# Baverne/VAE-CYCLEGAN-Implementation

Hardware: AMD Instinct MI355X
Metric: train images/sec (256x256 VAE-CycleGAN step) (higher is better)
Workload: dtype f32; 1 GPU; cyclevaegan unpaired, 3x256x256 synthetic summer<->winter, per-GPU batch 8, latent 64 (BASELINE.json configs[3]/[4]); per_gpu_batch=8, global_batch=8, image_size=256, latent_dim=64, parallelism=dp1, init=random (reference init statistics)

## Files before the change

vae-cyclegan-implementation_amd/csrc/conv_wino.hip:

```cpp
#include "vcg_common.h"
#ifdef VCG_STAMP
#include <stdlib.h>
#endif

#define WINO_U_SHIFT 2
#define WINO_V_SHIFT 2
int vcg_gemm_planes_batched(const void* APlanes, const void* BtPlanes, float* C, int rows, int K, int N, int batches, const VcgAmax& amax_a,
                            const VcgAmax& amax_b, hipStream_t st, uint32_t* amax_a_keep);

struct WinoP {
  const float* x;
  const float* m;
  const float* bias;
  float* y;
  int N, H, W, Cin, Cout, Hl, Wl, ups, reflect, act, cout_log;
  int th, tw, T, Kc;
  int off;
  FastDiv fd_k4, fd_tw, fd_thtw, fd_c4, fd_co4;
  unsigned long long* amax_slot;
  uint32_t amax_gen;
  VcgAmax amax_x;
  unsigned short* vplanes;
  const float* pre_mean;
  const float* pre_rstd;
  int pre_act;
};
__device__ __forceinline__ float4 wino_pre_apply(const float4& v, const float4& mu, const float4& rs, int act) {
  return make_float4(act_apply((v.x - mu.x) * rs.x, act), act_apply((v.y - mu.y) * rs.y, act), act_apply((v.z - mu.z) * rs.z, act),
                     act_apply((v.w - mu.w) * rs.w, act));
}

__device__ __forceinline__ float4 f4sub(const float4& a, const float4& b) { return make_float4(a.x - b.x, a.y - b.y, a.z - b.z, a.w - b.w); }
__device__ __forceinline__ float4 f4sum(const float4& a, const float4& b) { return make_float4(a.x + b.x, a.y + b.y, a.z + b.z, a.w + b.w); }

__global__ __launch_bounds__(256) void k_wino_in_planes(WinoP p) {
  float sc, inv;
  vcg_scale_of(vcg_amax_bits(p.amax_x), p.amax_x.shift, sc, inv);
  const uint32_t k4n = (uint32_t)p.Kc / 4;
  const size_t total = (size_t)p.T * k4n;
  const size_t KB = (size_t)p.Kc / 32;
  for (size_t idx = (size_t)blockIdx.x * blockDim.x + threadIdx.x; idx < total; idx += (size_t)gridDim.x * blockDim.x) {
// ... 377 lines not shown
  const size_t plane = (size_t)p.T * p.Cout;
  for (size_t idx = (size_t)blockIdx.x * blockDim.x + threadIdx.x; idx < total; idx += (size_t)gridDim.x * blockDim.x) {
    const uint32_t t = (uint32_t)(idx / c4n);
    const int co = (int)(idx - (size_t)t * c4n) * 4;
    const uint32_t n = fd_div(t, p.fd_thtw);
    const uint32_t rem = t - n * (uint32_t)(p.th * p.tw);
    const uint32_t ty = fd_div(rem, p.fd_tw);
    const int tx = (int)(rem - ty * (uint32_t)p.tw);
    const float* base = dy + (((size_t)n * p.Hl + 2 * ty) * p.Wl + 2 * tx) * p.Cout + co;
    const float4 y00 = *reinterpret_cast<const float4*>(base);
    const float4 y01 = *reinterpret_cast<const float4*>(base + p.Cout);
    const float4 y10 = *reinterpret_cast<const float4*>(base + (size_t)p.Wl * p.Cout);
    const float4 y11 = *reinterpret_cast<const float4*>(base + (size_t)p.Wl * p.Cout + p.Cout);
    const float4 zero = make_float4(0.f, 0.f, 0.f, 0.f);
    float4 z[4][2];
    z[0][0] = y00;              z[0][1] = y01;
    z[1][0] = f4sum(y00, y10);  z[1][1] = f4sum(y01, y11);
    z[2][0] = f4sub(y00, y10);  z[2][1] = f4sub(y01, y11);
    z[3][0] = f4sub(zero, y10); z[3][1] = f4sub(zero, y11);
    float* mb = dm + (size_t)t * p.Cout + co;
#pragma unroll
    for (int a = 0; a < 4; ++a) {
      const float4 o1 = f4sum(z[a][0], z[a][1]), o2 = f4sub(z[a][0], z[a][1]);
      *reinterpret_cast<float4*>(mb + (size_t)(a * 4 + 0) * plane) = z[a][0];
      *reinterpret_cast<float4*>(mb + (size_t)(a * 4 + 1) * plane) = o1;
      *reinterpret_cast<float4*>(mb + (size_t)(a * 4 + 2) * plane) = o2;
      *reinterpret_cast<float4*>(mb + (size_t)(a * 4 + 3) * plane) = f4sub(zero, z[a][1]);
      amax = max(amax, max(max(vcg_abs_bits4(z[a][0]), vcg_abs_bits4(z[a][1])), max(vcg_abs_bits4(o1), vcg_abs_bits4(o2))));
    }
  }
  if (p.amax_slot) vcg_amax_publish(amax, p.amax_slot, p.amax_gen, amax_red);
}

constexpr int WT_PITCH = 34;
__device__ __forceinline__ void wino_tr_store(unsigned short* __restrict__ sh, const float4* __restrict__ o4, float inv, int tl, int q,
                                              unsigned short* __restrict__ dst, size_t xi_stride, size_t row0, int TB, int tb) {
#pragma unroll
  for (int x = 0; x < 4; ++x) {
    uint2 h, l;
    split4h(o4[x], inv, h, l);
    const unsigned short hv[4] = {(unsigned short)h.x, (unsigned short)(h.x >> 16), (unsigned short)h.y, (unsigned short)(h.y >> 16)};
    const unsigned short lv[4] = {(unsigned short)l.x, (unsigned short)(l.x >> 16), (unsigned short)l.y, (unsigned short)(l.y >> 16)};
#pragma unroll
    for (int e = 0; e < 4; ++e) {
      sh[((x * 2 + 0) * 32 + 4 * q + e) * WT_PITCH + tl] = hv[e];
      sh[((x * 2 + 1) * 32 + 4 * q + e) * WT_PITCH + tl] = lv[e];
    }
  }
  __syncthreads();
  {
    const int pc = threadIdx.x & 1, c = (threadIdx.x >> 1) & 31, x = threadIdx.x >> 6;
    const uint32_t* src = reinterpret_cast<const uint32_t*>(sh + ((x * 2 + pc) * 32 + c) * WT_PITCH);
    uint4 v[4];
#pragma unroll
    for (int j = 0; j < 4; ++j) v[j] = make_uint4(src[4 * j], src[4 * j + 1], src[4 * j + 2], src[4 * j + 3]);
    unsigned short* o = dst + (size_t)x * xi_stride + ((row0 + c) * TB + tb) * VCG_PBLK + pc * 32;
#pragma unroll
    for (int j = 0; j < 4; ++j) *reinterpret_cast<uint4*>(o + 8 * j) = v[j];
  }
  __syncthreads();
}
__global__ __launch_bounds__(256) void k_wino_in_tr(WinoP p, unsigned short* __restrict__ vt) {
  __shared__ __attribute__((aligned(16))) unsigned short sh[4 * 2 * 32 * WT_PITCH];
  float sc, inv;
  vcg_scale_of(vcg_amax_bits(p.amax_x), p.amax_x.shift, sc, inv);
  const int tl = threadIdx.x >> 3, q = threadIdx.x & 7;
  const uint32_t t = blockIdx.x * 32 + tl;
  const uint32_t k4 = blockIdx.y * 8 + q;
  const uint32_t ph = fd_div(k4, p.fd_c4);
  const int c = (int)(k4 - ph * (uint32_t)(p.Cin / 4)) * 4;
  const int pi = (int)(ph >> 1), pj = (int)(ph & 1);
  const uint32_t n = fd_div(t, p.fd_thtw);
  const uint32_t rem = t - n * (uint32_t)(p.th * p.tw);
  const uint32_t ty = fd_div(rem, p.fd_tw);
  const int tx = (int)(rem - ty * (uint32_t)p.tw);
  const float* xn = p.x + (size_t)n * p.H * p.W * p.Cin;
  float4 pmu = make_float4(0.f, 0.f, 0.f, 0.f), prs = pmu;
  if (p.pre_mean) {
    pmu = *reinterpret_cast<const float4*>(p.pre_mean + (size_t)n * p.Cin + c);
    prs = *reinterpret_cast<const float4*>(p.pre_rstd + (size_t)n * p.Cin + c);
  }
  float4 d[4][4];
#pragma unroll
  for (int r = 0; r < 4; ++r) {
    int ih = 2 * (int)ty - p.off + r;
    bool okh = true;
    if (p.reflect) ih = reflect_idx(ih, p.Hl);
    else okh = ih >= 0 && ih < p.Hl;
#pragma unroll
    for (int s = 0; s < 4; ++s) {
      int iw = 2 * tx - p.off + s;
      bool ok = okh;
      if (p.reflect) iw = reflect_idx(iw, p.Wl);
      else ok = ok && iw >= 0 && iw < p.Wl;
      d[r][s] = ok ? *reinterpret_cast<const float4*>(xn + ((size_t)(ih * p.ups + pi) * p.W + (iw * p.ups + pj)) * p.Cin + c)
                   : make_float4(0.f, 0.f, 0.f, 0.f);
      if (p.pre_mean && ok) d[r][s] = wino_pre_apply(d[r][s], pmu, prs, p.pre_act);
    }
  }
  float4 e[4][4];
#pragma unroll
  for (int s = 0; s < 4; ++s) {
    e[0][s] = f4sub(d[0][s], d[2][s]);
    e[1][s] = f4sum(d[1][s], d[2][s]);
    e[2][s] = f4sub(d[2][s], d[1][s]);
    e[3][s] = f4sub(d[1][s], d[3][s]);
  }
  const uint32_t k = k4 * 4;
  const size_t KB = (size_t)p.Kc / 32;
  const int TB = p.T / 32;
#pragma unroll
  for (int a = 0; a < 4; ++a) {
    const float4 o[4] = {f4sub(e[a][0], e[a][2]), f4sum(e[a][1], e[a][2]), f4sub(e[a][2], e[a][1]), f4sub(e[a][1], e[a][3])};
    if (p.vplanes) {
      unsigned short* vb = p.vplanes + ((size_t)t * KB + k / 32) * VCG_PBLK + (k & 31);
      const size_t plane = (size_t)p.T * KB * VCG_PBLK;
#pragma unroll
      for (int b = 0; b < 4; ++b) {
        uint2 h, l;
        split4h(o[b], inv, h, l);
        unsigned short* w = vb + (size_t)(a * 4 + b) * plane;
        *reinterpret_cast<uint2*>(w) = h;
        *reinterpret_cast<uint2*>(w + 32) = l;
      }
    }
    if (vt) wino_tr_store(sh, o, inv, tl, q, vt + (size_t)(a * 4) * p.Kc * TB * VCG_PBLK, (size_t)p.Kc * TB * VCG_PBLK, (size_t)blockIdx.y * 32, TB, (int)blockIdx.x);
  }
}
__global__ __launch_bounds__(256) void k_wino_dy_tr(const float* __restrict__ dy, unsigned short* __restrict__ dmt, WinoP p) {
  __shared__ __attribute__((aligned(16))) unsigned short sh[4 * 2 * 32 * WT_PITCH];
  float sc, inv;
  vcg_scale_of(vcg_amax_bits(p.amax_x), p.amax_x.shift, sc, inv);
  const int tl = threadIdx.x >> 3, q = threadIdx.x & 7;
  const uint32_t t = blockIdx.x * 32 + tl;
  const int co = ((int)blockIdx.y * 8 + q) * 4;
  const uint32_t n = fd_div(t, p.fd_thtw);
  const uint32_t rem = t - n * (uint32_t)(p.th * p.tw);
  const uint32_t ty = fd_div(rem, p.fd_tw);
  const int tx = (int)(rem - ty * (uint32_t)p.tw);
  const float* base = dy + (((size_t)n * p.Hl + 2 * ty) * p.Wl + 2 * tx) * p.Cout + co;
  const float4 y00 = *reinterpret_cast<const float4*>(base);
  const float4 y01 = *reinterpret_cast<const float4*>(base + p.Cout);
  const float4 y10 = *reinterpret_cast<const float4*>(base + (size_t)p.Wl * p.Cout);
  const float4 y11 = *reinterpret_cast<const float4*>(base + (size_t)p.Wl * p.Cout + p.Cout);
  const float4 zero = make_float4(0.f, 0.f, 0.f, 0.f);
  float4 z[4][2];
  z[0][0] = y00;              z[0][1] = y01;
  z[1][0] = f4sum(y00, y10);  z[1][1] = f4sum(y01, y11);
  z[2][0] = f4sub(y00, y10);  z[2][1] = f4sub(y01, y11);
  z[3][0] = f4sub(zero, y10); z[3][1] = f4sub(zero, y11);
  const int TB = p.T / 32;
#pragma unroll
  for (int a = 0; a < 4; ++a) {
    const float4 o[4] = {z[a][0], f4sum(z[a][0], z[a][1]), f4sub(z[a][0], z[a][1]), f4sub(zero, z[a][1])};
    wino_tr_store(sh, o, inv, tl, q, dmt + (size_t)(a * 4) * p.Cout * TB * VCG_PBLK, (size_t)p.Cout * TB * VCG_PBLK, (size_t)blockIdx.y * 32, TB, (int)blockIdx.x);
  }
}

static int wino_blocks(size_t work) {
  size_t b = (work + 255) / 256;
  if (b > 8192) b = 8192;
  return b < 1 ? 1 : (int)b;
}

bool vcg_wino_weight_ok(const ConvGeom& g) {
  return g.KH == 3 && g.KW == 3 && g.stride == 1 && g.pad == 1 && g.ups * g.ups * g.Cin >= 128 && g.Cout >= 64 &&
         g.Cin % 4 == 0 && g.Cout % 64 == 0 && (g.ups * g.ups * g.Cin) % 64 == 0;
}
static bool wino_map_ok(const ConvGeom& g) {
  if (!vcg_wino_weight_ok(g)) return false;
#ifdef VCG_STAMP
  if (getenv("VCG_NO_WINOGRAD")) return false;
#endif
  return !(g.Ho < 4 || g.Wo < 4 || (g.Ho & 1) || (g.Wo & 1));
}
bool vcg_wino_fwd_ok(const ConvGeom& g) {
  if (!wino_map_ok(g)) return false;
  const unsigned long long T = (unsigned long long)g.N * (g.Ho / 2) * (g.Wo / 2);
  const unsigned long long Kc = (unsigned long long)g.ups * g.ups * g.Cin;
  if (Kc * g.Cout < (unsigned long long)kWinoGateFwd * (Kc + g.Cout)) return false;
  return T * Kc * 4 < (1ull << 31) && T * g.Cout * 4 < (1ull << 31) && T * Kc * 16 < (1ull << 32);
}
size_t vcg_wino_weight_floats(const ConvGeom& g) { return (size_t)16 * g.ups * g.ups * g.Cin * g.Cout * VCG_NP / 2; }
size_t vcg_wino_fwd_workspace(const ConvGeom& g) {
  const size_t T = (size_t)g.N * (g.Ho / 2) * (g.Wo / 2);
  return (size_t)16 * T * ((size_t)g.ups * g.ups * g.Cin + g.Cout) * sizeof(float) + 512;
}
int vcg_wino_weight(const ConvGeom& g, const float* w_oihw, float* u, const VcgAmax& amax_w, hipStream_t st) {
// ... 16 lines not shown
  p.fd_co4 = make_fastdiv((uint32_t)g.Cout / 4);
  p.off = 1;
  p.amax_slot = nullptr; p.amax_gen = 0;
  p.amax_x = vcg_amax_const(0); p.vplanes = nullptr;
  p.pre_mean = nullptr; p.pre_rstd = nullptr; p.pre_act = VCG_ACT_NONE;
  return p;
}

bool vcg_wino_wgrad_ok(const ConvGeom& g) {
  const long long kc = (long long)g.ups * g.ups * g.Cin;
  return vcg_wino_fwd_ok(g) && kc % 128 == 0 && kc * g.Cout >= kWinoGateWgrad * (kc + g.Cout);
}
bool vcg_wino_wgrad_tr_ok(const ConvGeom& g) {
  if (!vcg_wino_wgrad_ok(g)) return false;
  const long long kc = (long long)g.ups * g.ups * g.Cin, T = (long long)g.N * (g.Ho / 2) * (g.Wo / 2);
  return T % 32 == 0 && kc % 32 == 0 && g.Cout % 128 == 0 && kc >= 256 && ((kc + 255) / 256) * (g.Cout / 128) * 16 >= 192 &&
         16 * kc * T * VCG_NP < (1ll << 32) && 16 * (long long)g.Cout * T * VCG_NP < (1ll << 32);
}
size_t vcg_wino_wgrad_workspace(const ConvGeom& g) {
  const int T = g.N * (g.Ho / 2) * (g.Wo / 2);
  return vcg_wino_fwd_workspace(g) + vcg_wino_wgrad_core_workspace(g, T);
}
static size_t wino_v_floats(const ConvGeom& g) { return (size_t)16 * g.N * (g.Ho / 2) * (g.Wo / 2) * g.ups * g.ups * g.Cin; }
size_t vcg_wino_saved_floats(const ConvGeom& g) { return vcg_wino_wgrad_ok(g) ? wino_v_floats(g) + 16 : 0; }
int vcg_wino_wgrad(const ConvGeom& g, const float* x, const float* dy, float* gw_oihw, void* ws, size_t ws_bytes, hipStream_t st,
                   const float* v_saved, uint64_t x_handle, uint64_t dy_handle) {
  VCG_CHECK_ARG(ws && ws_bytes >= vcg_wino_wgrad_workspace(g), "vcg_conv_wgrad: workspace too small for the Winograd path");
  WinoP p = wino_params(g);
  float* V = (float*)ws;
  float* dM = V + (((size_t)16 * p.T * p.Kc + 63) / 64) * 64;
  const size_t tbytes = vcg_wino_fwd_workspace(g);
  if (vcg_wino_wgrad_tr_ok(g)) {
    VcgAmax amax_v;
    const unsigned short* Vt;
    if (v_saved) {
      Vt = reinterpret_cast<const unsigned short*>(v_saved);
      amax_v = vcg_amax_stored(v_saved + wino_v_floats(g), WINO_V_SHIFT);
    } else {
      if (vcg_operand_amax(x, (size_t)g.N * g.H * g.W * g.Cin, x_handle, WINO_V_SHIFT, st, &amax_v)) return -2;
      p.x = x; p.amax_x = amax_v; p.vplanes = nullptr;
      hipLaunchKernelGGL(k_wino_in_tr, dim3(p.T / 32, p.Kc / 32), dim3(256), 0, st, p, (unsigned short*)V);
      Vt = reinterpret_cast<const unsigned short*>(V);
    }
    VcgAmax amax_d;
    if (vcg_operand_amax(dy, (size_t)g.N * g.Ho * g.Wo * g.Cout, dy_handle, WINO_V_SHIFT, st, &amax_d)) return -2;
    WinoP pd = p;
    pd.amax_x = amax_d;
    hipLaunchKernelGGL(k_wino_dy_tr, dim3(p.T / 32, g.Cout / 32), dim3(256), 0, st, dy, (unsigned short*)dM, pd);
    VCG_LAUNCH_CHECK("vcg_conv_wgrad(winograd transforms, transposed)");
    float* dU = reinterpret_cast<float*>((char*)ws + tbytes);
    if (vcg_gemm_planes_batched(Vt, dM, dU, p.Kc, p.T, g.Cout, 16, amax_v, amax_d, st, nullptr)) return -2;
    return vcg_wino_wgrad_reduce_one(g, dU, gw_oihw, st);
  }
  p.x = x;
  VcgAmax amax_v;
  if (v_saved) {
    V = const_cast<float*>(v_saved);
    amax_v = vcg_amax_stored(v_saved + wino_v_floats(g), WINO_V_SHIFT);
  } else {
    if (vcg_operand_amax(x, (size_t)g.N * g.H * g.W * g.Cin, x_handle, WINO_V_SHIFT, st, &amax_v)) return -2;
    p.amax_x = amax_v; p.vplanes = (unsigned short*)V;
    hipLaunchKernelGGL(k_wino_in_planes, dim3(wino_blocks((size_t)p.T * p.Kc / 4)), dim3(256), 0, st, p);
  }
  const VcgAmaxOut ad = vcg_amax_new(st);
  p.amax_slot = ad.slot; p.amax_gen = ad.gen;
  hipLaunchKernelGGL(k_wino_dy, dim3(wino_blocks((size_t)p.T * g.Cout / 4)), dim3(256), 0, st, dy, dM, p);
  VCG_LAUNCH_CHECK("vcg_conv_wgrad(winograd transforms)");
  return vcg_wino_wgrad_core(g, V, dM, p.T, gw_oihw, (char*)ws + tbytes, ws_bytes - tbytes, st, amax_v, vcg_amax_in(ad));
}

bool vcg_wino_dgrad_ok(const ConvGeom& g) {
  if (!wino_map_ok(g)) return false;
  const long long kc = (long long)g.ups * g.ups * g.Cin;
  if (kc * g.Cout < kWinoGateDgrad * (kc + g.Cout)) return false;
  const unsigned long long Tp = (unsigned long long)g.N * (g.Ho / 2 + 1) * (g.Wo / 2 + 1);
  return Tp * kc * 4 < (1ull << 31) && Tp * g.Cout * 4 < (1ull << 31) && Tp * g.Cout * 16 < (1ull << 32);
}
size_t vcg_wino_dgrad_workspace(const ConvGeom& g) {
  const size_t Tp = (size_t)g.N * (g.Ho / 2 + 1) * (g.Wo / 2 + 1);
  const size_t kc = (size_t)g.ups * g.ups * g.Cin;
  return (size_t)16 * Tp * (kc + g.Cout) * sizeof(float) + 1024;
}
int vcg_wino_weight_dgrad(const ConvGeom& g, const float* w_oihw, float* ud, const VcgAmax& amax_w, hipStream_t st) {
  const size_t total = (size_t)g.ups * g.ups * g.Cin * g.Cout / 4;
// ... 24 lines not shown
  if (vcg_operand_amax(dy, (size_t)g.N * g.Ho * g.Wo * g.Cout, dy_handle, WINO_V_SHIFT, st, &ad)) return -2;
  p.amax_x = ad; p.vplanes = (unsigned short*)V;
  hipLaunchKernelGGL(k_wino_in_planes, dim3(wino_blocks((size_t)p.T * g.Cout / 4)), dim3(256), 0, st, p);
  VCG_LAUNCH_CHECK("vcg_conv_dgrad(winograd input transform)");
  if (vcg_gemm_planes_batched(V, ud, M, p.T, g.Cout, kc, 16, ad, vcg_amax_stored(w_amax, WINO_U_SHIFT), st, nullptr)) return -2;
  WinoP q = p;
  q.Kc = kc;
  hipLaunchKernelGGL(k_wino_out_fold, dim3(wino_blocks((size_t)p.T * kc / 4)), dim3(256), 0, st, (const float*)M, dx, q, g.Hl, g.Wl,
                     g.Cin, g.ups, g.reflect);
  VCG_LAUNCH_CHECK("vcg_conv_dgrad(winograd output transform)");
  return 0;
}

size_t vcg_wino_fwd_stats_doubles(const ConvGeom& g) {
  const NormPlan pl = vcg_norm_plan(g.N, (g.Ho / 2) * (g.Wo / 2), g.Cout);
  return (size_t)g.N * pl.nchunk * g.Cout * 2;
}
int vcg_wino_fwd(const ConvGeom& g, const float* x, const float* u, const void* w_amax, const float* bias, float* y, void* ws,
                 size_t ws_bytes, hipStream_t st, double* in_part, const VcgInStatsOut* stats, float* v_keep, uint64_t x_handle,
                 const VcgPre* pre) {
  VCG_CHECK_ARG(ws && ws_bytes >= vcg_wino_fwd_workspace(g), "vcg_conv_fwd: workspace too small for the Winograd path (%zu)",
                ws_bytes);
  WinoP p = wino_params(g);
  float* V = v_keep ? v_keep : (float*)ws;
  float* M = (float*)ws + (((size_t)16 * p.T * p.Kc + 63) / 64) * 64;
  p.x = x; p.m = M; p.bias = bias; p.y = y;
  uint32_t pre_bits = 0;
  if (pre && pre->mean) {
    p.pre_mean = pre->mean; p.pre_rstd = pre->rstd; p.pre_act = pre->act;
    const float bound = sqrtf((float)g.H * (float)g.W);
    memcpy(&pre_bits, &bound, 4);
  }
  uint32_t* const keep_word = v_keep ? reinterpret_cast<uint32_t*>(v_keep + wino_v_floats(g)) : nullptr;
  if (v_keep && vcg_wino_wgrad_tr_ok(g)) {
    VcgAmax ax;
    if (pre_bits) ax = vcg_amax_const(pre_bits, WINO_V_SHIFT);
    else if (vcg_operand_amax(x, (size_t)g.N * g.H * g.W * g.Cin, x_handle, WINO_V_SHIFT, st, &ax)) return -2;
    V = (float*)ws;
    p.amax_x = ax; p.vplanes = (unsigned short*)V;
    hipLaunchKernelGGL(k_wino_in_tr, dim3(p.T / 32, p.Kc / 32), dim3(256), 0, st, p, (unsigned short*)v_keep);
    VCG_LAUNCH_CHECK("vcg_conv_fwd(winograd input transform, + transposed)");
    if (vcg_gemm_planes_batched(V, u, M, p.T, p.Kc, g.Cout, 16, ax, vcg_amax_stored(w_amax, WINO_U_SHIFT), st, keep_word)) return -2;
  } else {
    VcgAmax ax;
    if (pre_bits) ax = vcg_amax_const(pre_bits, WINO_V_SHIFT);
    else if (vcg_operand_amax(x, (size_t)g.N * g.H * g.W * g.Cin, x_handle, WINO_V_SHIFT, st, &ax)) return -2;
    p.amax_x = ax; p.vplanes = (unsigned short*)V;
    hipLaunchKernelGGL(k_wino_in_planes, dim3(wino_blocks((size_t)p.T * p.Kc / 4)), dim3(256), 0, st, p);
    VCG_LAUNCH_CHECK("vcg_conv_fwd(winograd input transform)");
    if (vcg_gemm_planes_batched(V, u, M, p.T, p.Kc, g.Cout, 16, ax, vcg_amax_stored(w_amax, WINO_U_SHIFT), st, keep_word)) return -2;
  }
  if (in_part) {
    const NormPlan pl = vcg_norm_plan(g.N, p.th * p.tw, g.Cout);
    hipLaunchKernelGGL(k_wino_out_stats, dim3(pl.nchunk, g.N, pl.cgroups), dim3(256), 0, st, p, in_part, pl);
    VCG_LAUNCH_CHECK("vcg_conv_fwd(winograd output transform)");
    return vcg_in_finalize(in_part, stats->mean, stats->rstd, g.N, stats->HW, g.Cout, pl.nchunk, stats->eps, st);
  } else {
    hipLaunchKernelGGL(k_wino_out, dim3(wino_blocks((size_t)p.T * g.Cout / 4)), dim3(256), 0, st, p);
  }
  VCG_LAUNCH_CHECK("vcg_conv_fwd(winograd output transform)");
  return 0;
}
```

vae-cyclegan-implementation_amd/csrc/gemm_split.hip:

```cpp
#include "vcg_common.h"

typedef unsigned int u32x4g __attribute__((ext_vector_type(4)));

struct GemmSplitP {
  const float* a;
  const float* bt;
  float* c;
  int rows, K, N;
  uint32_t a_bytes, b_bytes;
  uint32_t a_bstride, b_bstride;
  size_t c_bstride;
  VcgAmax amax_a, amax_b;
  uint32_t* amax_a_keep;
};

#define GS_OOB 0x80000000u

template <int BN>
__global__ __launch_bounds__(256, 2) void k_gemm_split(GemmSplitP p) {
  constexpr int BM = 128, NI = BN / 64, MI = 2;
  __shared__ __attribute__((aligned(16))) unsigned char As[VCG_NP][BM * 64];
  __shared__ __attribute__((aligned(16))) unsigned char Bs[VCG_NP][BN * 64];
  const int tid = threadIdx.x, lane = tid & 63, wid = tid >> 6;
  const int wm = wid >> 1, wn = wid & 1, l31 = lane & 31, lh = lane >> 5;
// ... 116 lines not shown

struct GdSrd { uint32_t x, y, z, w; };
typedef uint32_t gd_u32x4 __attribute__((ext_vector_type(4)));
__device__ __forceinline__ gd_u32x4 gd_srd(const void* ptr, uint32_t bytes) {
  const uint64_t a = (uint64_t)ptr;
  gd_u32x4 r;
  r.x = __builtin_amdgcn_readfirstlane((uint32_t)a);
  r.y = __builtin_amdgcn_readfirstlane((uint32_t)(a >> 32) & 0xFFFFu);
  r.z = __builtin_amdgcn_readfirstlane(bytes);
  r.w = 0x00020000u;
  return r;
}
__device__ __forceinline__ void gd_dma16(gd_u32x4 srd, uint32_t lds_dst, uint32_t voff) {
  uint32_t keep;
  asm volatile("s_mov_b32 %0, m0\n\ts_mov_b32 m0, %2\n\ts_nop 0\n\tbuffer_load_dwordx4 %1, %3, 0 offen lds\n\ts_mov_b32 m0, %0"
               : "=&s"(keep) : "v"(voff), "s"(lds_dst), "s"(srd) : "memory");
}
__device__ __forceinline__ void gd_barrier() {
  asm volatile("s_waitcnt lgkmcnt(0)\n\ts_barrier" ::: "memory");
}
constexpr int GD_BM = 256, GD_BN = 128;
constexpr int GD_A_BYTES = GD_BM * VCG_PBYTES, GD_B_BYTES = GD_BN * VCG_PBYTES;
constexpr int GD_STAGE = GD_A_BYTES + GD_B_BYTES;
constexpr int GD_STAGES = 3;
#ifdef VCG_GD_STAMP
__device__ unsigned long long* g_gd_stamp = nullptr;
int vcg_gd_set_stamp(void* buf) { return hipMemcpyToSymbol(HIP_SYMBOL(g_gd_stamp), &buf, sizeof(buf)) == hipSuccess ? 0 : -1; }
#define GD_T() (__builtin_amdgcn_sched_barrier(0), __builtin_amdgcn_s_memtime())
#define GD_ACC(slot, t0) do { const unsigned long long t1__ = GD_T(); gd_acc[slot] += t1__ - (t0); (t0) = t1__; } while (0)
#else
#define GD_T() 0ull
#define GD_ACC(slot, t0) do { } while (0)
#endif
__global__ __launch_bounds__(512, 1) void k_gemm_planes_dma(GemmSplitP p) {
  __shared__ __attribute__((aligned(1024))) unsigned char smem[GD_STAGES * GD_STAGE];
  const int tid = threadIdx.x, lane = tid & 63, wid = tid >> 6;
  const int wm = wid >> 1, wn = wid & 1;
  float sa_, inv_a, sb_, inv_b;
  {
    const uint32_t abits = vcg_amax_bits(p.amax_a);
    vcg_scale_of(abits, p.amax_a.shift, sa_, inv_a);
    vcg_scale_of(vcg_amax_bits(p.amax_b), p.amax_b.shift, sb_, inv_b);
    if (p.amax_a_keep && tid == 0 && blockIdx.x == 0 && blockIdx.y == 0 && blockIdx.z == 0) *p.amax_a_keep = abits;
  }
  int mt, nt, zb;
  {
    const uint32_t per = gridDim.x * gridDim.y, nwg = per * gridDim.z;
    const uint32_t gid = blockIdx.x + gridDim.x * (blockIdx.y + gridDim.y * blockIdx.z);
    const uint32_t q = nwg >> 3, r = nwg & 7, xcd = gid & 7;
    const uint32_t swz = (xcd < r ? xcd * (q + 1) : r * (q + 1) + (xcd - r) * q) + (gid >> 3);
    zb = (int)(swz / per);
    const uint32_t l = swz - (uint32_t)zb * per;
    mt = (int)(l / gridDim.y);
    nt = (int)(l - (uint32_t)mt * gridDim.y);
  }
  const int m0 = mt * GD_BM, n0 = nt * GD_BN;
  const gd_u32x4 ra = gd_srd((const unsigned short*)p.a + (size_t)zb * p.a_bstride, p.a_bytes),
                 rb = gd_srd((const unsigned short*)p.bt + (size_t)zb * p.b_bstride, p.b_bytes);
  const int KB = p.K / 32;
  const int drow = lane >> 3, dslot = lane & 7;
  uint32_t aoff[4], boff[2];
#pragma unroll
  for (int h = 0; h < 4; ++h) {
    const int rl = (wid + 8 * h) * 8 + drow;
    const int r = m0 + rl;
    aoff[h] = r < p.rows ? (uint32_t)((size_t)r * KB * VCG_PBYTES + ((dslot ^ ((rl >> 1) & 7)) << 4)) : GS_OOB;
  }
#pragma unroll
  for (int h = 0; h < 2; ++h) {
    const int rl = (wid + 8 * h) * 8 + drow;
    boff[h] = (uint32_t)((size_t)(n0 + rl) * KB * VCG_PBYTES + ((dslot ^ ((rl >> 1) & 7)) << 4));
  }
  const uint32_t lds0 = (uint32_t)(uintptr_t)(__attribute__((address_space(3))) unsigned char*)smem;
  auto issue_one = [&](int stage, int kt, int q) {
    const uint32_t sbase = __builtin_amdgcn_readfirstlane(lds0 + (uint32_t)stage * GD_STAGE);
    const uint32_t ko = (uint32_t)kt * VCG_PBYTES;
    if (q < 4) gd_dma16(ra, __builtin_amdgcn_readfirstlane(sbase + (uint32_t)((wid + 8 * q) * 1024)), aoff[q] != GS_OOB ? aoff[q] + ko : GS_OOB);
    else gd_dma16(rb, __builtin_amdgcn_readfirstlane(sbase + (uint32_t)(GD_A_BYTES + (wid + 8 * (q - 4)) * 1024)), boff[q - 4] + ko);
  };
  auto issue = [&](int stage, int kt) {
#pragma unroll
    for (int q = 0; q < 6; ++q) issue_one(stage, kt, q);
  };

  f32x4 acc16[4][4], lo16[4][4];
#pragma unroll
  for (int i = 0; i < 4; ++i)
#pragma unroll
    for (int j = 0; j < 4; ++j)
#pragma unroll
      for (int e = 0; e < 4; ++e) acc16[i][j][e] = lo16[i][j][e] = 0.f;
  const int r16 = lane & 15, kq = lane >> 4;
  uint32_t fa16[4], fb16[4];
  int sa16[4], sb16[4];
#pragma unroll
  for (int i = 0; i < 4; ++i) { const int r = wm * 64 + i * 16 + r16; fa16[i] = (uint32_t)(r * VCG_PBYTES); sa16[i] = (r >> 1) & 7; }
#pragma unroll
  for (int j = 0; j < 4; ++j) { const int r = wn * 64 + j * 16 + r16; fb16[j] = (uint32_t)(GD_A_BYTES + r * VCG_PBYTES); sb16[j] = (r >> 1) & 7; }

  const int nkt = KB;
#ifdef VCG_GD_STAMP
  unsigned long long gd_acc[8] = {0, 0, 0, 0, 0, 0, 0, 0};
  const unsigned long long gd_start = GD_T(), gd_rt0 = __builtin_amdgcn_s_memrealtime();
#endif
  issue(0, 0);
  if (nkt > 1) issue(1, 1);
  unsigned long long gd_t = GD_T();
  (void)gd_t;
  f16x8 a16[VCG_NP][4], b16[VCG_NP][4];
  auto read16 = [&](int kt) {
    const unsigned char* st = smem + (kt % GD_STAGES) * GD_STAGE;
#pragma unroll
    for (int pc = 0; pc < VCG_NP; ++pc) {
#pragma unroll
      for (int i = 0; i < 4; ++i)
        a16[pc][i] = *reinterpret_cast<const f16x8*>(st + fa16[i] + (((pc * 4 + kq) ^ sa16[i]) << 4));
#pragma unroll
      for (int j = 0; j < 4; ++j)
        b16[pc][j] = *reinterpret_cast<const f16x8*>(st + fb16[j] + (((pc * 4 + kq) ^ sb16[j]) << 4));
    }
  };
  auto mma16 = [&](int dkt) {
    const bool more = dkt < nkt;
    const int nstage = dkt % GD_STAGES;
    int q = 0;
#pragma unroll
    for (int i = 0; i < 4; ++i)
#pragma unroll
      for (int j = 0; j < 4; ++j) {
        f32x4 c = lo16[i][j];
        c = __builtin_amdgcn_mfma_f32_16x16x32_f16(a16[1][i], b16[0][j], c, 0, 0, 0);
        c = __builtin_amdgcn_mfma_f32_16x16x32_f16(a16[0][i], b16[1][j], c, 0, 0, 0);
        lo16[i][j] = c;
        acc16[i][j] = __builtin_amdgcn_mfma_f32_16x16x32_f16(a16[0][i], b16[0][j], acc16[i][j], 0, 0, 0);
        if ((j & 1) && q < 6) {
          __builtin_amdgcn_sched_barrier(0);
          if (more) issue_one(nstage, dkt, q);
          __builtin_amdgcn_sched_barrier(0);
          ++q;
        }
      }
  };
  const bool late = wid >= 4;
  for (int kt = 0; kt < nkt; ++kt) {
    if (kt + 1 < nkt) asm volatile("s_waitcnt vmcnt(6)" ::: "memory");
    else asm volatile("s_waitcnt vmcnt(0)" ::: "memory");
    GD_ACC(0, gd_t);
    gd_barrier();
    GD_ACC(1, gd_t);
    if (!late) {
      read16(kt);
      mma16(kt + 2);
// ... 42 lines not shown
    split4h(*reinterpret_cast<const float4*>(x + e), inv, h, l);
    unsigned short* o = bp + (row * (K / 32) + k / 32) * VCG_PBLK + (k & 31);
    *reinterpret_cast<uint2*>(o) = h;
    *reinterpret_cast<uint2*>(o + 32) = l;
  }
}
int vcg_split_planes(const float* x, void* bp, size_t rows, int K, const VcgAmax& amax, hipStream_t st) {
  VCG_CHECK_ARG(K % 32 == 0, "vcg_split_planes: K must be a multiple of 32");
  const size_t quads = rows * K / 4;
  size_t blocks = (quads + 255) / 256; if (blocks > 8192) blocks = 8192;
  hipLaunchKernelGGL(k_split_planes, dim3((unsigned)blocks), dim3(256), 0, st, x, (unsigned short*)bp, quads, K, amax);
  VCG_LAUNCH_CHECK("vcg_split_planes");
  return 0;
}

int vcg_gemm_planes_batched(const void* APlanes, const void* BtPlanes, float* C, int rows, int K, int N, int batches, const VcgAmax& amax_a,
                            const VcgAmax& amax_b, hipStream_t st, uint32_t* amax_a_keep) {
  VCG_CHECK_ARG(K % 32 == 0 && N % 64 == 0 && rows > 0, "vcg_gemm_planes_batched: bad shape rows=%d K=%d N=%d", rows, K, N);
  VCG_CHECK_ARG((unsigned long long)rows * K * 2 * VCG_NP < (1ull << 31) && (unsigned long long)N * K * 2 * VCG_NP < (1ull << 31),
                "vcg_gemm_planes_batched: operand extents must stay below 2 GiB per batch");
  VCG_CHECK_ARG((unsigned long long)rows * K * VCG_NP * (unsigned long long)batches < (1ull << 32) &&
                    (unsigned long long)N * K * VCG_NP * (unsigned long long)batches < (1ull << 32),
                "vcg_gemm_planes_batched: batch stride overflow");
  GemmSplitP p;
  p.a = (const float*)APlanes; p.bt = (const float*)BtPlanes; p.c = C; p.rows = rows; p.K = K; p.N = N;
  p.a_bytes = (uint32_t)((size_t)rows * K * 2 * VCG_NP); p.b_bytes = (uint32_t)((size_t)N * K * 2 * VCG_NP);
  p.a_bstride = (uint32_t)((size_t)rows * K * VCG_NP); p.b_bstride = (uint32_t)((size_t)N * K * VCG_NP);
  p.c_bstride = (size_t)rows * N;
  p.amax_a = amax_a; p.amax_b = amax_b; p.amax_a_keep = amax_a_keep;
  const int bn = (N % 128 == 0) ? 128 : 64;
  if (bn == 128 && rows >= 256) {
    dim3 grid((rows + GD_BM - 1) / GD_BM, N / GD_BN, batches);
    VcgProfScope prof("k_gemm_planes_dma", 2.0 * rows * (double)K * N * batches, st);
    hipLaunchKernelGGL(k_gemm_planes_dma, grid, dim3(512), 0, st, p);
    VCG_LAUNCH_CHECK("vcg_gemm_planes_batched(dma)");
    return 0;
  }
  dim3 grid((rows + 127) / 128, N / bn, batches);
  VcgProfScope prof(bn == 128 ? "k_gemm_split<128, planes>" : "k_gemm_split<64, planes>", 2.0 * rows * (double)K * N * batches, st);
  if (bn == 128) hipLaunchKernelGGL((k_gemm_split<128>), grid, dim3(256), 0, st, p);
  else hipLaunchKernelGGL((k_gemm_split<64>), grid, dim3(256), 0, st, p);
  VCG_LAUNCH_CHECK("vcg_gemm_planes_batched");
  return 0;
}
```

Before: 249.3 images/s.

## Replace transposed Winograd transforms with TN GEMM using LDS transpose reads

Removes the shared-memory transpose kernels (k_wino_in_tr, k_wino_dy_tr) that wrote transposed copies of Winograd operands for the weight-gradient GEMM. The input and dy transforms now write plain plane layout, and a new TN variant of the DMA GEMM reads K-major tiles through ds_read_tr16 LDS transpose instructions. This also lets the forward pass drop the extra transposed V copy it saved for wgrad. The risk is lower GEMM efficiency from the new address swizzle and transpose reads, and a tighter shape restriction (rows%32, N%GD_BN) on the TN path.

```diff
diff --git a/vae-cyclegan-implementation_amd/csrc/conv_wino.hip b/vae-cyclegan-implementation_amd/csrc/conv_wino.hip
--- a/vae-cyclegan-implementation_amd/csrc/conv_wino.hip
+++ b/vae-cyclegan-implementation_amd/csrc/conv_wino.hip
@@ -7,6 +7,8 @@
 #define WINO_V_SHIFT 2
 int vcg_gemm_planes_batched(const void* APlanes, const void* BtPlanes, float* C, int rows, int K, int N, int batches, const VcgAmax& amax_a,
                             const VcgAmax& amax_b, hipStream_t st, uint32_t* amax_a_keep);
+int vcg_gemm_planes_tn_batched(const void* APlanes, const void* BPlanes, float* C, int rows, int K, int N, int batches, const VcgAmax& amax_a,
+                               const VcgAmax& amax_b, hipStream_t st);
 
 struct WinoP {
   const float* x;
@@ -450,128 +452,44 @@
   if (p.amax_slot) vcg_amax_publish(amax, p.amax_slot, p.amax_gen, amax_red);
 }
 
-constexpr int WT_PITCH = 34;
-__device__ __forceinline__ void wino_tr_store(unsigned short* __restrict__ sh, const float4* __restrict__ o4, float inv, int tl, int q,
-                                              unsigned short* __restrict__ dst, size_t xi_stride, size_t row0, int TB, int tb) {
-#pragma unroll
-  for (int x = 0; x < 4; ++x) {
-    uint2 h, l;
-    split4h(o4[x], inv, h, l);
-    const unsigned short hv[4] = {(unsigned short)h.x, (unsigned short)(h.x >> 16), (unsigned short)h.y, (unsigned short)(h.y >> 16)};
-    const unsigned short lv[4] = {(unsigned short)l.x, (unsigned short)(l.x >> 16), (unsigned short)l.y, (unsigned short)(l.y >> 16)};
-#pragma unroll
-    for (int e = 0; e < 4; ++e) {
-      sh[((x * 2 + 0) * 32 + 4 * q + e) * WT_PITCH + tl] = hv[e];
-      sh[((x * 2 + 1) * 32 + 4 * q + e) * WT_PITCH + tl] = lv[e];
-    }
-  }
-  __syncthreads();
-  {
-    const int pc = threadIdx.x & 1, c = (threadIdx.x >> 1) & 31, x = threadIdx.x >> 6;
-    const uint32_t* src = reinterpret_cast<const uint32_t*>(sh + ((x * 2 + pc) * 32 + c) * WT_PITCH);
-    uint4 v[4];
-#pragma unroll
-    for (int j = 0; j < 4; ++j) v[j] = make_uint4(src[4 * j], src[4 * j + 1], src[4 * j + 2], src[4 * j + 3]);
-    unsigned short* o = dst + (size_t)x * xi_stride + ((row0 + c) * TB + tb) * VCG_PBLK + pc * 32;
-#pragma unroll
-    for (int j = 0; j < 4; ++j) *reinterpret_cast<uint4*>(o + 8 * j) = v[j];
-  }
-  __syncthreads();
-}
-__global__ __launch_bounds__(256) void k_wino_in_tr(WinoP p, unsigned short* __restrict__ vt) {
-  __shared__ __attribute__((aligned(16))) unsigned short sh[4 * 2 * 32 * WT_PITCH];
+__global__ __launch_bounds__(256) void k_wino_dy_planes(const float* __restrict__ dy, unsigned short* __restrict__ dmp, WinoP p) {
   float sc, inv;
   vcg_scale_of(vcg_amax_bits(p.amax_x), p.amax_x.shift, sc, inv);
-  const int tl = threadIdx.x >> 3, q = threadIdx.x & 7;
-  const uint32_t t = blockIdx.x * 32 + tl;
-  const uint32_t k4 = blockIdx.y * 8 + q;
-  const uint32_t ph = fd_div(k4, p.fd_c4);
-  const int c = (int)(k4 - ph * (uint32_t)(p.Cin / 4)) * 4;
-  const int pi = (int)(ph >> 1), pj = (int)(ph & 1);
-  const uint32_t n = fd_div(t, p.fd_thtw);
-  const uint32_t rem = t - n * (uint32_t)(p.th * p.tw);
-  const uint32_t ty = fd_div(rem, p.fd_tw);
-  const int tx = (int)(rem - ty * (uint32_t)p.tw);
-  const float* xn = p.x + (size_t)n * p.H * p.W * p.Cin;
-  float4 pmu = make_float4(0.f, 0.f, 0.f, 0.f), prs = pmu;
-  if (p.pre_mean) {
-    pmu = *reinterpret_cast<const float4*>(p.pre_mean + (size_t)n * p.Cin + c);
-    prs = *reinterpret_cast<const float4*>(p.pre_rstd + (size_t)n * p.Cin + c);
-  }
-  float4 d[4][4];
-#pragma unroll
-  for (int r = 0; r < 4; ++r) {
-    int ih = 2 * (int)ty - p.off + r;
-    bool okh = true;
-    if (p.reflect) ih = reflect_idx(ih, p.Hl);
-    else okh = ih >= 0 && ih < p.Hl;
-#pragma unroll
-    for (int s = 0; s < 4; ++s) {
-      int iw = 2 * tx - p.off + s;
-      bool ok = okh;
-      if (p.reflect) iw = reflect_idx(iw, p.Wl);
-      else ok = ok && iw >= 0 && iw < p.Wl;
-      d[r][s] = ok ? *reinterpret_cast<const float4*>(xn + ((size_t)(ih * p.ups + pi) * p.W + (iw * p.ups + pj)) * p.Cin + c)
-                   : make_float4(0.f, 0.f, 0.f, 0.f);
-      if (p.pre_mean && ok) d[r][s] = wino_pre_apply(d[r][s], pmu, prs, p.pre_act);
-    }
-  }
-  float4 e[4][4];
-#pragma unroll
-  for (int s = 0; s < 4; ++s) {
-    e[0][s] = f4sub(d[0][s], d[2][s]);
-    e[1][s] = f4sum(d[1][s], d[2][s]);
-    e[2][s] = f4sub(d[2][s], d[1][s]);
-    e[3][s] = f4sub(d[1][s], d[3][s]);
-  }
-  const uint32_t k = k4 * 4;
-  const size_t KB = (size_t)p.Kc / 32;
-  const int TB = p.T / 32;
-#pragma unroll
-  for (int a = 0; a < 4; ++a) {
-    const float4 o[4] = {f4sub(e[a][0], e[a][2]), f4sum(e[a][1], e[a][2]), f4sub(e[a][2], e[a][1]), f4sub(e[a][1], e[a][3])};
-    if (p.vplanes) {
-      unsigned short* vb = p.vplanes + ((size_t)t * KB + k / 32) * VCG_PBLK + (k & 31);
-      const size_t plane = (size_t)p.T * KB * VCG_PBLK;
+  const uint32_t c4n = (uint32_t)p.Cout / 4;
+  const size_t total = (size_t)p.T * c4n;
+  const size_t CB = (size_t)p.Cout / 32;
+  const size_t plane = (size_t)p.T * CB * VCG_PBLK;
+  for (size_t idx = (size_t)blockIdx.x * blockDim.x + threadIdx.x; idx < total; idx += (size_t)gridDim.x * blockDim.x) {
+    const uint32_t t = (uint32_t)(idx / c4n);
+    const uint32_t co = (uint32_t)(idx - (size_t)t * c4n) * 4;
+    const uint32_t n = fd_div(t, p.fd_thtw);
+    const uint32_t rem = t - n * (uint32_t)(p.th * p.tw);
+    const uint32_t ty = fd_div(rem, p.fd_tw);
+    const int tx = (int)(rem - ty * (uint32_t)p.tw);
+    const float* base = dy + (((size_t)n * p.Hl + 2 * ty) * p.Wl + 2 * tx) * p.Cout + co;
+    const float4 y00 = *reinterpret_cast<const float4*>(base);
+    const float4 y01 = *reinterpret_cast<const float4*>(base + p.Cout);
+    const float4 y10 = *reinterpret_cast<const float4*>(base + (size_t)p.Wl * p.Cout);
+    const float4 y11 = *reinterpret_cast<const float4*>(base + (size_t)p.Wl * p.Cout + p.Cout);
+    const float4 zero = make_float4(0.f, 0.f, 0.f, 0.f);
+    float4 z[4][2];
+    z[0][0] = y00;              z[0][1] = y01;
+    z[1][0] = f4sum(y00, y10);  z[1][1] = f4sum(y01, y11);
+    z[2][0] = f4sub(y00, y10);  z[2][1] = f4sub(y01, y11);
+    z[3][0] = f4sub(zero, y10); z[3][1] = f4sub(zero, y11);
+    unsigned short* mb = dmp + ((size_t)t * CB + co / 32) * VCG_PBLK + (co & 31);
+#pragma unroll
+    for (int a = 0; a < 4; ++a) {
+      const float4 o[4] = {z[a][0], f4sum(z[a][0], z[a][1]), f4sub(z[a][0], z[a][1]), f4sub(zero, z[a][1])};
 #pragma unroll
       for (int b = 0; b < 4; ++b) {
         uint2 h, l;
         split4h(o[b], inv, h, l);
-        unsigned short* w = vb + (size_t)(a * 4 + b) * plane;
-        *reinterpret_cast<uint2*>(w) = h;
-        *reinterpret_cast<uint2*>(w + 32) = l;
-      }
-    }
-    if (vt) wino_tr_store(sh, o, inv, tl, q, vt + (size_t)(a * 4) * p.Kc * TB * VCG_PBLK, (size_t)p.Kc * TB * VCG_PBLK, (size_t)blockIdx.y * 32, TB, (int)blockIdx.x);
-  }
-}
-__global__ __launch_bounds__(256) void k_wino_dy_tr(const float* __restrict__ dy, unsigned short* __restrict__ dmt, WinoP p) {
-  __shared__ __attribute__((aligned(16))) unsigned short sh[4 * 2 * 32 * WT_PITCH];
-  float sc, inv;
-  vcg_scale_of(vcg_amax_bits(p.amax_x), p.amax_x.shift, sc, inv);
-  const int tl = threadIdx.x >> 3, q = threadIdx.x & 7;
-  const uint32_t t = blockIdx.x * 32 + tl;
-  const int co = ((int)blockIdx.y * 8 + q) * 4;
-  const uint32_t n = fd_div(t, p.fd_thtw);
-  const uint32_t rem = t - n * (uint32_t)(p.th * p.tw);
-  const uint32_t ty = fd_div(rem, p.fd_tw);
-  const int tx = (int)(rem - ty * (uint32_t)p.tw);
-  const float* base = dy + (((size_t)n * p.Hl + 2 * ty) * p.Wl + 2 * tx) * p.Cout + co;
-  const float4 y00 = *reinterpret_cast<const float4*>(base);
-  const float4 y01 = *reinterpret_cast<const float4*>(base + p.Cout);
-  const float4 y10 = *reinterpret_cast<const float4*>(base + (size_t)p.Wl * p.Cout);
-  const float4 y11 = *reinterpret_cast<const float4*>(base + (size_t)p.Wl * p.Cout + p.Cout);
-  const float4 zero = make_float4(0.f, 0.f, 0.f, 0.f);
-  float4 z[4][2];
-  z[0][0] = y00;              z[0][1] = y01;
-  z[1][0] = f4sum(y00, y10);  z[1][1] = f4sum(y01, y11);
-  z[2][0] = f4sub(y00, y10);  z[2][1] = f4sub(y01, y11);
-  z[3][0] = f4sub(zero, y10); z[3][1] = f4sub(zero, y11);
-  const int TB = p.T / 32;
-#pragma unroll
-  for (int a = 0; a < 4; ++a) {
-    const float4 o[4] = {z[a][0], f4sum(z[a][0], z[a][1]), f4sub(z[a][0], z[a][1]), f4sub(zero, z[a][1])};
-    wino_tr_store(sh, o, inv, tl, q, dmt + (size_t)(a * 4) * p.Cout * TB * VCG_PBLK, (size_t)p.Cout * TB * VCG_PBLK, (size_t)blockIdx.y * 32, TB, (int)blockIdx.x);
+        unsigned short* q = mb + (size_t)(a * 4 + b) * plane;
+        *reinterpret_cast<uint2*>(q) = h;
+        *reinterpret_cast<uint2*>(q + 32) = l;
+      }
+    }
   }
 }
 
@@ -654,24 +572,24 @@
   const size_t tbytes = vcg_wino_fwd_workspace(g);
   if (vcg_wino_wgrad_tr_ok(g)) {
     VcgAmax amax_v;
-    const unsigned short* Vt;
+    const float* Vp;
     if (v_saved) {
-      Vt = reinterpret_cast<const unsigned short*>(v_saved);
+      Vp = v_saved;
       amax_v = vcg_amax_stored(v_saved + wino_v_floats(g), WINO_V_SHIFT);
     } else {
       if (vcg_operand_amax(x, (size_t)g.N * g.H * g.W * g.Cin, x_handle, WINO_V_SHIFT, st, &amax_v)) return -2;
-      p.x = x; p.amax_x = amax_v; p.vplanes = nullptr;
-      hipLaunchKernelGGL(k_wino_in_tr, dim3(p.T / 32, p.Kc / 32), dim3(256), 0, st, p, (unsigned short*)V);
-      Vt = reinterpret_cast<const unsigned short*>(V);
+      p.x = x; p.amax_x = amax_v; p.vplanes = (unsigned short*)V;
+      hipLaunchKernelGGL(k_wino_in_planes, dim3(wino_blocks((size_t)p.T * p.Kc / 4)), dim3(256), 0, st, p);
+      Vp = V;
     }
     VcgAmax amax_d;
     if (vcg_operand_amax(dy, (size_t)g.N * g.Ho * g.Wo * g.Cout, dy_handle, WINO_V_SHIFT, st, &amax_d)) return -2;
     WinoP pd = p;
     pd.amax_x = amax_d;
-    hipLaunchKernelGGL(k_wino_dy_tr, dim3(p.T / 32, g.Cout / 32), dim3(256), 0, st, dy, (unsigned short*)dM, pd);
-    VCG_LAUNCH_CHECK("vcg_conv_wgrad(winograd transforms, transposed)");
+    hipLaunchKernelGGL(k_wino_dy_planes, dim3(wino_blocks((size_t)p.T * g.Cout / 4)), dim3(256), 0, st, dy, (unsigned short*)dM, pd);
+    VCG_LAUNCH_CHECK("vcg_conv_wgrad(winograd transforms, planes)");
     float* dU = reinterpret_cast<float*>((char*)ws + tbytes);
-    if (vcg_gemm_planes_batched(Vt, dM, dU, p.Kc, p.T, g.Cout, 16, amax_v, amax_d, st, nullptr)) return -2;
+    if (vcg_gemm_planes_tn_batched(Vp, dM, dU, p.Kc, p.T, g.Cout, 16, amax_v, amax_d, st)) return -2;
     return vcg_wino_wgrad_reduce_one(g, dU, gw_oihw, st);
   }
   p.x = x;
@@ -762,24 +680,13 @@
     memcpy(&pre_bits, &bound, 4);
   }
   uint32_t* const keep_word = v_keep ? reinterpret_cast<uint32_t*>(v_keep + wino_v_floats(g)) : nullptr;
-  if (v_keep && vcg_wino_wgrad_tr_ok(g)) {
-    VcgAmax ax;
-    if (pre_bits) ax = vcg_amax_const(pre_bits, WINO_V_SHIFT);
-    else if (vcg_operand_amax(x, (size_t)g.N * g.H * g.W * g.Cin, x_handle, WINO_V_SHIFT, st, &ax)) return -2;
-    V = (float*)ws;
-    p.amax_x = ax; p.vplanes = (unsigned short*)V;
-    hipLaunchKernelGGL(k_wino_in_tr, dim3(p.T / 32, p.Kc / 32), dim3(256), 0, st, p, (unsigned short*)v_keep);
-    VCG_LAUNCH_CHECK("vcg_conv_fwd(winograd input transform, + transposed)");
-    if (vcg_gemm_planes_batched(V, u, M, p.T, p.Kc, g.Cout, 16, ax, vcg_amax_stored(w_amax, WINO_U_SHIFT), st, keep_word)) return -2;
-  } else {
-    VcgAmax ax;
-    if (pre_bits) ax = vcg_amax_const(pre_bits, WINO_V_SHIFT);
-    else if (vcg_operand_amax(x, (size_t)g.N * g.H * g.W * g.Cin, x_handle, WINO_V_SHIFT, st, &ax)) return -2;
-    p.amax_x = ax; p.vplanes = (unsigned short*)V;
-    hipLaunchKernelGGL(k_wino_in_planes, dim3(wino_blocks((size_t)p.T * p.Kc / 4)), dim3(256), 0, st, p);
-    VCG_LAUNCH_CHECK("vcg_conv_fwd(winograd input transform)");
-    if (vcg_gemm_planes_batched(V, u, M, p.T, p.Kc, g.Cout, 16, ax, vcg_amax_stored(w_amax, WINO_U_SHIFT), st, keep_word)) return -2;
-  }
+  VcgAmax ax;
+  if (pre_bits) ax = vcg_amax_const(pre_bits, WINO_V_SHIFT);
+  else if (vcg_operand_amax(x, (size_t)g.N * g.H * g.W * g.Cin, x_handle, WINO_V_SHIFT, st, &ax)) return -2;
+  p.amax_x = ax; p.vplanes = (unsigned short*)V;
+  hipLaunchKernelGGL(k_wino_in_planes, dim3(wino_blocks((size_t)p.T * p.Kc / 4)), dim3(256), 0, st, p);
+  VCG_LAUNCH_CHECK("vcg_conv_fwd(winograd input transform)");
+  if (vcg_gemm_planes_batched(V, u, M, p.T, p.Kc, g.Cout, 16, ax, vcg_amax_stored(w_amax, WINO_U_SHIFT), st, keep_word)) return -2;
   if (in_part) {
     const NormPlan pl = vcg_norm_plan(g.N, p.th * p.tw, g.Cout);
     hipLaunchKernelGGL(k_wino_out_stats, dim3(pl.nchunk, g.N, pl.cgroups), dim3(256), 0, st, p, in_part, pl);
diff --git a/vae-cyclegan-implementation_amd/csrc/gemm_split.hip b/vae-cyclegan-implementation_amd/csrc/gemm_split.hip
--- a/vae-cyclegan-implementation_amd/csrc/gemm_split.hip
+++ b/vae-cyclegan-implementation_amd/csrc/gemm_split.hip
@@ -172,6 +172,15 @@
 #define GD_T() 0ull
 #define GD_ACC(slot, t0) do { } while (0)
 #endif
+typedef short gd_s16x4 __attribute__((ext_vector_type(4)));
+__device__ __forceinline__ f16x8 gd_tr_frag(uint32_t a, uint32_t kstride4) {
+  const gd_s16x4 lo = __builtin_amdgcn_ds_read_tr16_b64_v4i16((__attribute__((address_space(3))) gd_s16x4*)(uintptr_t)a);
+  const gd_s16x4 hi = __builtin_amdgcn_ds_read_tr16_b64_v4i16((__attribute__((address_space(3))) gd_s16x4*)(uintptr_t)(a + kstride4));
+  typedef short gd_s16x8 __attribute__((ext_vector_type(8)));
+  const gd_s16x8 v = {lo[0], lo[1], lo[2], lo[3], hi[0], hi[1], hi[2], hi[3]};
+  return __builtin_bit_cast(f16x8, v);
+}
+template <bool TN>
 __global__ __launch_bounds__(512, 1) void k_gemm_planes_dma(GemmSplitP p) {
   __shared__ __attribute__((aligned(1024))) unsigned char smem[GD_STAGES * GD_STAGE];
   const int tid = threadIdx.x, lane = tid & 63, wid = tid >> 6;
@@ -202,21 +211,34 @@
   uint32_t aoff[4], boff[2];
 #pragma unroll
   for (int h = 0; h < 4; ++h) {
-    const int rl = (wid + 8 * h) * 8 + drow;
-    const int r = m0 + rl;
-    aoff[h] = r < p.rows ? (uint32_t)((size_t)r * KB * VCG_PBYTES + ((dslot ^ ((rl >> 1) & 7)) << 4)) : GS_OOB;
+    if constexpr (TN) {
+      const int kl = wid + 8 * h;
+      const int ch = lane ^ (((kl & 3) | (((kl >> 3) & 1) << 2)) << 1);
+      aoff[h] = m0 + 4 * ch < p.rows ? (uint32_t)((size_t)kl * p.rows * 4 + (size_t)m0 * 4 + ch * 16) : GS_OOB;
+    } else {
+      const int rl = (wid + 8 * h) * 8 + drow;
+      const int r = m0 + rl;
+      aoff[h] = r < p.rows ? (uint32_t)((size_t)r * KB * VCG_PBYTES + ((dslot ^ ((rl >> 1) & 7)) << 4)) : GS_OOB;
+    }
   }
 #pragma unroll
   for (int h = 0; h < 2; ++h) {
-    const int rl = (wid + 8 * h) * 8 + drow;
-    boff[h] = (uint32_t)((size_t)(n0 + rl) * KB * VCG_PBYTES + ((dslot ^ ((rl >> 1) & 7)) << 4));
+    if constexpr (TN) {
+      const int kl = 2 * (wid + 8 * h) + (lane >> 5);
+      const int ch = (lane & 31) ^ (((kl & 3) | (((kl >> 3) & 1) << 2)) << 1);
+      boff[h] = (uint32_t)((size_t)kl * p.N * 4 + (size_t)n0 * 4 + ch * 16);
+    } else {
+      const int rl = (wid + 8 * h) * 8 + drow;
+      boff[h] = (uint32_t)((size_t)(n0 + rl) * KB * VCG_PBYTES + ((dslot ^ ((rl >> 1) & 7)) << 4));
+    }
   }
   const uint32_t lds0 = (uint32_t)(uintptr_t)(__attribute__((address_space(3))) unsigned char*)smem;
   auto issue_one = [&](int stage, int kt, int q) {
     const uint32_t sbase = __builtin_amdgcn_readfirstlane(lds0 + (uint32_t)stage * GD_STAGE);
-    const uint32_t ko = (uint32_t)kt * VCG_PBYTES;
+    const uint32_t ko = TN ? (uint32_t)kt * 128u * (uint32_t)p.rows : (uint32_t)kt * VCG_PBYTES;
+    const uint32_t kob = TN ? (uint32_t)kt * 128u * (uint32_t)p.N : ko;
     if (q < 4) gd_dma16(ra, __builtin_amdgcn_readfirstlane(sbase + (uint32_t)((wid + 8 * q) * 1024)), aoff[q] != GS_OOB ? aoff[q] + ko : GS_OOB);
-    else gd_dma16(rb, __builtin_amdgcn_readfirstlane(sbase + (uint32_t)(GD_A_BYTES + (wid + 8 * (q - 4)) * 1024)), boff[q - 4] + ko);
+    else gd_dma16(rb, __builtin_amdgcn_readfirstlane(sbase + (uint32_t)(GD_A_BYTES + (wid + 8 * (q - 4)) * 1024)), boff[q - 4] + kob);
   };
   auto issue = [&](int stage, int kt) {
 #pragma unroll
@@ -237,6 +259,12 @@
   for (int i = 0; i < 4; ++i) { const int r = wm * 64 + i * 16 + r16; fa16[i] = (uint32_t)(r * VCG_PBYTES); sa16[i] = (r >> 1) & 7; }
 #pragma unroll
   for (int j = 0; j < 4; ++j) { const int r = wn * 64 + j * 16 + r16; fb16[j] = (uint32_t)(GD_A_BYTES + r * VCG_PBYTES); sb16[j] = (r >> 1) & 7; }
+  uint32_t ta16 = 0, tb16 = 0;
+  if constexpr (TN) {
+    const int tq = (lane >> 2) & 3, tp = lane & 3, tk = 8 * kq + tq, tf = tq | ((kq & 1) << 2);
+    ta16 = lds0 + (uint32_t)(tk * 1024 + wm * 256 + (tf << 5) + tp * 8);
+    tb16 = lds0 + (uint32_t)(GD_A_BYTES + tk * 512 + wn * 256 + (tf << 5) + tp * 8);
+  }
 
   const int nkt = KB;
 #ifdef VCG_GD_STAMP
@@ -250,14 +278,20 @@
   f16x8 a16[VCG_NP][4], b16[VCG_NP][4];
   auto read16 = [&](int kt) {
     const unsigned char* st = smem + (kt % GD_STAGES) * GD_STAGE;
+    const uint32_t sta = ta16 + (uint32_t)((kt % GD_STAGES) * GD_STAGE), stb = tb16 + (uint32_t)((kt % GD_STAGES) * GD_STAGE);
+    (void)st; (void)sta; (void)stb;
 #pragma unroll
     for (int pc = 0; pc < VCG_NP; ++pc) {
 #pragma unroll
-      for (int i = 0; i < 4; ++i)
-        a16[pc][i] = *reinterpret_cast<const f16x8*>(st + fa16[i] + (((pc * 4 + kq) ^ sa16[i]) << 4));
-#pragma unroll
-      for (int j = 0; j < 4; ++j)
-        b16[pc][j] = *reinterpret_cast<const f16x8*>(st + fb16[j] + (((pc * 4 + kq) ^ sb16[j]) << 4));
+      for (int i = 0; i < 4; ++i) {
+        if constexpr (TN) a16[pc][i] = gd_tr_frag(sta ^ (uint32_t)((((i >> 1) * 4 + pc * 2 + (i & 1))) << 5), 4 * 1024);
+        else a16[pc][i] = *reinterpret_cast<const f16x8*>(st + fa16[i] + (((pc * 4 + kq) ^ sa16[i]) << 4));
+      }
+#pragma unroll
+      for (int j = 0; j < 4; ++j) {
+        if constexpr (TN) b16[pc][j] = gd_tr_frag(stb ^ (uint32_t)((((j >> 1) * 4 + pc * 2 + (j & 1))) << 5), 4 * 512);
+        else b16[pc][j] = *reinterpret_cast<const f16x8*>(st + fb16[j] + (((pc * 4 + kq) ^ sb16[j]) << 4));
+      }
     }
   };
   auto mma16 = [&](int dkt) {
@@ -366,7 +400,7 @@
   if (bn == 128 && rows >= 256) {
     dim3 grid((rows + GD_BM - 1) / GD_BM, N / GD_BN, batches);
     VcgProfScope prof("k_gemm_planes_dma", 2.0 * rows * (double)K * N * batches, st);
-    hipLaunchKernelGGL(k_gemm_planes_dma, grid, dim3(512), 0, st, p);
+    hipLaunchKernelGGL(k_gemm_planes_dma<false>, grid, dim3(512), 0, st, p);
     VCG_LAUNCH_CHECK("vcg_gemm_planes_batched(dma)");
     return 0;
   }
@@ -377,3 +411,24 @@
   VCG_LAUNCH_CHECK("vcg_gemm_planes_batched");
   return 0;
 }
+
+int vcg_gemm_planes_tn_batched(const void* APlanes, const void* BPlanes, float* C, int rows, int K, int N, int batches, const VcgAmax& amax_a,
+                               const VcgAmax& amax_b, hipStream_t st) {
+  VCG_CHECK_ARG(K % 32 == 0 && K > 0 && N % GD_BN == 0 && rows % 32 == 0 && rows > 0, "vcg_gemm_planes_tn_batched: bad shape rows=%d K=%d N=%d", rows, K, N);
+  VCG_CHECK_ARG((unsigned long long)rows * K * 2 * VCG_NP < (1ull << 31) && (unsigned long long)N * K * 2 * VCG_NP < (1ull << 31),
+                "vcg_gemm_planes_tn_batched: operand extents must stay below 2 GiB per batch");
+  VCG_CHECK_ARG((unsigned long long)rows * K * VCG_NP * (unsigned long long)batches < (1ull << 32) &&
+                    (unsigned long long)N * K * VCG_NP * (unsigned long long)batches < (1ull << 32),
+                "vcg_gemm_planes_tn_batched: batch stride overflow");
+  GemmSplitP p;
+  p.a = (const float*)APlanes; p.bt = (const float*)BPlanes; p.c = C; p.rows = rows; p.K = K; p.N = N;
+  p.a_bytes = (uint32_t)((size_t)rows * K * 2 * VCG_NP); p.b_bytes = (uint32_t)((size_t)N * K * 2 * VCG_NP);
+  p.a_bstride = (uint32_t)((size_t)rows * K * VCG_NP); p.b_bstride = (uint32_t)((size_t)N * K * VCG_NP);
+  p.c_bstride = (size_t)rows * N;
+  p.amax_a = amax_a; p.amax_b = amax_b; p.amax_a_keep = nullptr;
+  dim3 grid((rows + GD_BM - 1) / GD_BM, N / GD_BN, batches);
+  VcgProfScope prof("k_gemm_planes_dma", 2.0 * rows * (double)K * N * batches, st);
+  hipLaunchKernelGGL(k_gemm_planes_dma<true>, grid, dim3(512), 0, st, p);
+  VCG_LAUNCH_CHECK("vcg_gemm_planes_tn_batched");
+  return 0;
+}
```

Result: slower. 242.4 images/s (-2.7%).
